# facebookresearch/seamless_communication

Measured on AMD Instinct MI355X. Metric: S2ST utterances/sec (and real-time factor), seamlessM4T_v2_large, 10 s audio, higher is better.
Workload: dtype f32 activations x f16 weights, f32 accumulate

## Files before the change

### seamless_communication_amd/csrc/k_attn.hip

```cpp
#include <cstdlib>

#include "kernels.h"

namespace sc {

static constexpr int HD = 64;

static constexpr int MQ = 128;
static constexpr int MKV = 32;
static constexpr int KS = 68;
typedef _Float16 a16_h8 __attribute__((ext_vector_type(8)));
typedef _Float16 a16_h4 __attribute__((ext_vector_type(4)));
static constexpr int KH_LD = 72;
static constexpr int VT_LD = 40;

__device__ __forceinline__ void a16_split8(const float* x, a16_h8& hi, a16_h8& lo) {
#pragma unroll
    for (int e = 0; e < 8; ++e) {
        const _Float16 h = (_Float16)x[e];
        hi[e] = h;
        lo[e] = (_Float16)(x[e] - (float)h);
    }
}

template <int MODE>
__global__ __launch_bounds__(256) void attn_mfma16_kernel(AttnArgs p) {
    constexpr bool SHAW = MODE == 1;
    constexpr bool RELPOS = MODE == 2;
    typedef float f16v __attribute__((ext_vector_type(16)));
    typedef float f4v __attribute__((ext_vector_type(4)));
    extern __shared__ __attribute__((aligned(16))) float smem[];
    _Float16* sKh = reinterpret_cast<_Float16*>(smem);
    _Float16* sKl = sKh + MKV * KH_LD;
    _Float16* sVh = sKl + MKV * KH_LD;
    _Float16* sVl = sVh + HD * VT_LD;
    float* sQR = smem + 4 * 32 * KS;
    float* sT = smem + 4 * 32 * KS;
    float* sR = smem;

    const int tid = threadIdx.x, lane = tid & 63, wave = tid >> 6;
    const int ql = lane & 31, hh = lane >> 5;
    int qb = blockIdx.x, h = blockIdx.y, n = blockIdx.z;
    {
        const int gx = gridDim.x, bh_all = gridDim.y * gridDim.z;
        if ((bh_all & 7) == 0) {
            const int L = blockIdx.x + gx * (blockIdx.y + gridDim.y * blockIdx.z);
            const int bh = (L / (8 * gx)) * 8 + (L & 7);
            qb = (L >> 3) % gx;
            h = bh % gridDim.y;
            n = bh / gridDim.y;
        }
    }
    const int q0 = qb * MQ + wave * 32;
    const int qi = q0 + ql;
    const int kv_len = p.kv_lens ? min(p.kv_lens[n], p.Skv) : p.Skv;
    const int shift = p.Skv - p.Sq;
    const int qabs = qi + shift;
    const int npos = p.rel_left + 1 + p.rel_right;
    const int sq_n = p.row_off ? kv_len : p.Sq;
    const int64_t qbase = p.row_off ? (int64_t)p.row_off[n] : (int64_t)n * p.Sq;
    const int64_t kvbase = p.row_off ? (int64_t)p.row_off[n] : (int64_t)n * p.Skv;
    if (p.row_off && qb * MQ >= kv_len) return;
    const bool qok = qi < sq_n;
    const float* qrow = p.q + (qbase + (qok ? qi : 0)) * p.ldq + h * HD;

    if (SHAW) {
        float qreg[32];
#pragma unroll
        for (int g = 0; g < 8; ++g) {
            f4v v = {0.f, 0.f, 0.f, 0.f};
            if (qok) v = *reinterpret_cast<const f4v*>(qrow + 8 * g + 4 * hh);
            qreg[4 * g + 0] = v[0];
            qreg[4 * g + 1] = v[1];
            qreg[4 * g + 2] = v[2];
            qreg[4 * g + 3] = v[3];
        }
        for (int idx = tid; idx < npos * (HD / 4); idx += 256) {
            const int r = idx >> 4, c4 = idx & 15;
            *reinterpret_cast<f4v*>(&sR[r * KS + c4 * 4]) = *reinterpret_cast<const f4v*>(p.rel_k + r * HD + c4 * 4);
        }
        __syncthreads();
#pragma unroll 1
        for (int f = 0; f < 3; ++f) {
            if (f * 32 >= npos) break;
            f16v qr;
#pragma unroll
            for (int r = 0; r < 16; ++r) qr[r] = 0.f;
#pragma unroll
            for (int g = 0; g < 8; ++g) {
                const f4v r4 = *reinterpret_cast<const f4v*>(&sR[(f * 32 + ql) * KS + 8 * g + 4 * hh]);
                qr = __builtin_amdgcn_mfma_f32_32x32x2f32(r4[0], qreg[4 * g + 0], qr, 0, 0, 0);
                qr = __builtin_amdgcn_mfma_f32_32x32x2f32(r4[1], qreg[4 * g + 1], qr, 0, 0, 0);
                qr = __builtin_amdgcn_mfma_f32_32x32x2f32(r4[2], qreg[4 * g + 2], qr, 0, 0, 0);
                qr = __builtin_amdgcn_mfma_f32_32x32x2f32(r4[3], qreg[4 * g + 3], qr, 0, 0, 0);
            }
#pragma unroll
            for (int r = 0; r < 16; ++r) {
                const int e = f * 32 + (r & 3) + 8 * (r >> 2) + 4 * hh;
                if (e < npos) sQR[(wave * 32 + ql) * npos + e] = qr[r];
            }
        }
    }

    a16_h8 qh[4], qlo[4], qvh[RELPOS ? 4 : 1], qvl[RELPOS ? 4 : 1];
#pragma unroll
    for (int c = 0; c < 4; ++c) {
        float x[8];
#pragma unroll
        for (int e = 0; e < 8; ++e) x[e] = 0.f;
        if (qok) {
            const f4v v0 = *reinterpret_cast<const f4v*>(qrow + 16 * c + 8 * hh);
            const f4v v1 = *reinterpret_cast<const f4v*>(qrow + 16 * c + 8 * hh + 4);
#pragma unroll
            for (int e = 0; e < 4; ++e) {
                x[e] = v0[e];
                x[4 + e] = v1[e];
            }
        }
        if (RELPOS) {
            float xu[8], xv[8];
#pragma unroll
            for (int e = 0; e < 8; ++e) {
                xu[e] = x[e] + p.q_bias_u[h * HD + 16 * c + 8 * hh + e];
                xv[e] = x[e] + p.q_bias_v[h * HD + 16 * c + 8 * hh + e];
            }
            a16_split8(xu, qh[c], qlo[c]);
            a16_split8(xv, qvh[c], qvl[c]);
        } else {
            a16_split8(x, qh[c], qlo[c]);
        }
    }

    f16v o0, o1;
#pragma unroll
    for (int r = 0; r < 16; ++r) {
        o0[r] = 0.f;
        o1[r] = 0.f;
    }
    float m_i = -1e30f, l_i = 0.f;

    int k_end = kv_len;
    if (p.causal) k_end = min(k_end, qb * MQ + MQ - 1 + shift + 1);

    const int sr0 = tid >> 4, sc4 = tid & 15;
    f4v kf[2], vf[2];
    auto fetch = [&](int k0) {
#pragma unroll
        for (int u = 0; u < 2; ++u) {
            const int r = sr0 + 16 * u;
            kf[u] = f4v{0.f, 0.f, 0.f, 0.f};
            vf[u] = kf[u];
            if (k0 + r < kv_len) {
                const int64_t row = kvbase + k0 + r;
                kf[u] = *reinterpret_cast<const f4v*>(p.k + row * p.ldk + h * HD + sc4 * 4);
                vf[u] = *reinterpret_cast<const f4v*>(p.v + row * p.ldv + h * HD + sc4 * 4);
            }
        }
    };
    if (k_end > 0) fetch(0);

    for (int k0 = 0; k0 < k_end; k0 += MKV) {
        __syncthreads();
#pragma unroll
        for (int u = 0; u < 2; ++u) {
            const int r = sr0 + 16 * u;
            a16_h4 khi, klo, vhi, vlo;
#pragma unroll
            for (int e = 0; e < 4; ++e) {
                const _Float16 a = (_Float16)kf[u][e];
                khi[e] = a;
                klo[e] = (_Float16)(kf[u][e] - (float)a);
                const _Float16 b = (_Float16)vf[u][e];
                vhi[e] = b;
                vlo[e] = (_Float16)(vf[u][e] - (float)b);
            }
            *reinterpret_cast<a16_h4*>(&sKh[r * KH_LD + 4 * sc4]) = khi;
            *reinterpret_cast<a16_h4*>(&sKl[r * KH_LD + 4 * sc4]) = klo;
            const int w = r & 15;
            const int pos = (r & 16) + 8 * ((w >> 2) & 1) + (w & 3) + 4 * (w >> 3);
#pragma unroll
            for (int e = 0; e < 4; ++e) {
                sVh[(4 * sc4 + e) * VT_LD + pos] = vhi[e];
                sVl[(4 * sc4 + e) * VT_LD + pos] = vlo[e];
            }
        }
        if (k0 + MKV < k_end) fetch(k0 + MKV);
        __syncthreads();

        float qr[16];
        if (SHAW) {
            const float* qrow_t = sQR + (wave * 32 + ql) * npos;
            const int rel_max = k0 + (MKV - 1) - (q0 + shift);
            const int rel_min = k0 - (q0 + 31 + shift);
            if (rel_max <= -p.rel_left) {
                const float v = qrow_t[0];
#pragma unroll
                for (int r = 0; r < 16; ++r) qr[r] = v;
            } else if (rel_min >= p.rel_right) {
                const float v = qrow_t[npos - 1];
#pragma unroll
                for (int r = 0; r < 16; ++r) qr[r] = v;
            } else {
#pragma unroll
                for (int r = 0; r < 16; ++r) {
                    const int kj = k0 + (r & 3) + 8 * (r >> 2) + 4 * hh;
                    const int rel = max(-p.rel_left, min(p.rel_right, kj - qabs)) + p.rel_left;
                    qr[r] = qrow_t[rel];
                }
            }
        }
        if (RELPOS) {
            const int t0w = (p.Skv - 1) - (q0 + shift) + k0 - 31;
            const int t_max = 2 * p.Skv - 2;
            float* tw = sT + wave * (64 * 32);
#pragma unroll
            for (int blk = 0; blk < 2; ++blk) {
                const int trow = min(max(t0w + blk * 32 + ql, 0), t_max);
                const float* rrow = p.rp_table + (int64_t)trow * p.rp_ld + h * HD + 8 * hh;
                f4v ra[4][2];
#pragma unroll
                for (int c = 0; c < 4; ++c) {
                    ra[c][0] = *reinterpret_cast<const f4v*>(rrow + 16 * c);
                    ra[c][1] = *reinterpret_cast<const f4v*>(rrow + 16 * c + 4);
                }
                f16v tt;
#pragma unroll
                for (int r = 0; r < 16; ++r) tt[r] = 0.f;
#pragma unroll
                for (int c = 0; c < 4; ++c) {
                    float x[8];
#pragma unroll
                    for (int e = 0; e < 4; ++e) {
                        x[e] = ra[c][0][e];
                        x[4 + e] = ra[c][1][e];
                    }
                    a16_h8 rh, rl;
                    a16_split8(x, rh, rl);
                    tt = __builtin_amdgcn_mfma_f32_32x32x16_f16(rh, qvh[c], tt, 0, 0, 0);
                    tt = __builtin_amdgcn_mfma_f32_32x32x16_f16(rh, qvl[c], tt, 0, 0, 0);
                    tt = __builtin_amdgcn_mfma_f32_32x32x16_f16(rl, qvh[c], tt, 0, 0, 0);
                }
#pragma unroll
                for (int r = 0; r < 16; ++r) tw[(blk * 32 + (r & 3) + 8 * (r >> 2) + 4 * hh) * 32 + ql] = tt[r];
            }
#pragma unroll
            for (int r = 0; r < 16; ++r) {
                const int jl = (r & 3) + 8 * (r >> 2) + 4 * hh;
                qr[r] = tw[(jl - ql + 31) * 32 + ql];
            }
        }
        f16v st;
#pragma unroll
        for (int r = 0; r < 16; ++r) st[r] = 0.f;
#pragma unroll
        for (int c = 0; c < 4; ++c) {
            const a16_h8 kh = *reinterpret_cast<const a16_h8*>(&sKh[ql * KH_LD + 16 * c + 8 * hh]);
            const a16_h8 kl = *reinterpret_cast<const a16_h8*>(&sKl[ql * KH_LD + 16 * c + 8 * hh]);
            st = __builtin_amdgcn_mfma_f32_32x32x16_f16(kh, qh[c], st, 0, 0, 0);
            st = __builtin_amdgcn_mfma_f32_32x32x16_f16(kh, qlo[c], st, 0, 0, 0);
            st = __builtin_amdgcn_mfma_f32_32x32x16_f16(kl, qh[c], st, 0, 0, 0);
        }
        float mx = -INFINITY;
#pragma unroll
        for (int r = 0; r < 16; ++r) {
            const int kj = k0 + (r & 3) + 8 * (r >> 2) + 4 * hh;
            float sc = st[r];
            if (SHAW || RELPOS) sc += qr[r];
            const bool ok = (kj < kv_len) && (!p.causal || kj <= qabs);
            sc = sc * 0.125f + (ok ? 0.f : -INFINITY);
            st[r] = sc;
            mx = fmaxf(mx, sc);
        }
        mx = fmaxf(mx, __shfl_xor(mx, 32));
        const float m_new = fmaxf(m_i, mx);
        constexpr float LOG2E = 1.44269504088896340736f;
        const float alpha = __builtin_amdgcn_exp2f((m_i - m_new) * LOG2E);
        float rs = 0.f;
#pragma unroll
        for (int r = 0; r < 16; ++r) {
            const float pv = __builtin_amdgcn_exp2f((st[r] - m_new) * LOG2E);
            st[r] = pv;
            rs += pv;
        }
        rs += __shfl_xor(rs, 32);
        l_i = l_i * alpha + rs;
        m_i = m_new;
        if (__builtin_amdgcn_ballot_w64(alpha != 1.f) != 0) {
#pragma unroll
            for (int r = 0; r < 16; ++r) {
                o0[r] *= alpha;
                o1[r] *= alpha;
            }
        }
#pragma unroll
        for (int c = 0; c < 2; ++c) {
            float x[8];
#pragma unroll
            for (int e = 0; e < 8; ++e) x[e] = st[8 * c + e];
            a16_h8 ph, pl;
            a16_split8(x, ph, pl);
            const a16_h8 v0h = *reinterpret_cast<const a16_h8*>(&sVh[ql * VT_LD + 16 * c + 8 * hh]);
            const a16_h8 v0l = *reinterpret_cast<const a16_h8*>(&sVl[ql * VT_LD + 16 * c + 8 * hh]);
            const a16_h8 v1h = *reinterpret_cast<const a16_h8*>(&sVh[(32 + ql) * VT_LD + 16 * c + 8 * hh]);
            const a16_h8 v1l = *reinterpret_cast<const a16_h8*>(&sVl[(32 + ql) * VT_LD + 16 * c + 8 * hh]);
            o0 = __builtin_amdgcn_mfma_f32_32x32x16_f16(v0h, ph, o0, 0, 0, 0);
            o1 = __builtin_amdgcn_mfma_f32_32x32x16_f16(v1h, ph, o1, 0, 0, 0);
            o0 = __builtin_amdgcn_mfma_f32_32x32x16_f16(v0h, pl, o0, 0, 0, 0);
            o1 = __builtin_amdgcn_mfma_f32_32x32x16_f16(v1h, pl, o1, 0, 0, 0);
            o0 = __builtin_amdgcn_mfma_f32_32x32x16_f16(v0l, ph, o0, 0, 0, 0);
            o1 = __builtin_amdgcn_mfma_f32_32x32x16_f16(v1l, ph, o1, 0, 0, 0);
        }
    }

    __syncthreads();
    float* ot = smem + wave * (32 * KS);
    const float inv = l_i > 0.f ? 1.0f / l_i : 0.f;
#pragma unroll
    for (int r = 0; r < 16; ++r) {
        const int d = (r & 3) + 8 * (r >> 2) + 4 * hh;
        ot[ql * KS + d] = o0[r] * inv;
        ot[ql * KS + 32 + d] = o1[r] * inv;
    }
#pragma unroll
    for (int it = 0; it < 8; ++it) {
        const int row = it * 4 + (lane >> 4);
        const int c0 = (lane & 15) * 4;
        const int qq = q0 + row;
        const f4v of = *reinterpret_cast<const f4v*>(&ot[row * KS + c0]);
        if (qq >= sq_n) continue;
        if (p.out_hi) {
            const a16_h4 hi = __builtin_convertvector(of, a16_h4);
            const f4v back = __builtin_convertvector(hi, f4v);
            const int64_t off = (qbase + qq) * p.ldoh + h * HD + c0;
            *reinterpret_cast<a16_h4*>(p.out_hi + off) = hi;
            *reinterpret_cast<a16_h4*>(p.out_lo + off) = __builtin_convertvector(of - back, a16_h4);
        } else {
            *reinterpret_cast<f4v*>(p.out + (qbase + qq) * p.ldo + h * HD + c0) = of;
        }
    }
}

static bool g_attn_attr_set = false;

void launch_attention(const AttnArgs& a, hipStream_t s) {
    if (a.head_dim == 80) {
        launch_attention80(a, s);
        return;
    }
    if (a.head_dim == 128) {
        launch_attention128(a, s);
        return;
    }
    SC_CHECK(a.head_dim == HD, "attention: head_dim=%d (64, 80 and 128 exist)", a.head_dim);
    SC_CHECK(a.nb > 0 && a.heads > 0 && a.Sq > 0 && a.Skv > 0, "attention: empty problem");
    SC_CHECK(a.out || (a.out_hi && a.out_lo && a.ldoh % 4 == 0), "attention: no output");
    SC_CHECK(a.ldq % 4 == 0 && a.ldk % 4 == 0 && a.ldv % 4 == 0 && a.ldo % 4 == 0 && (reinterpret_cast<uintptr_t>(a.out) & 15) == 0,
             "attention: row strides must be multiples of 4 and the output 16-byte aligned");
    const int npos = a.rel_left + 1 + a.rel_right;
    SC_CHECK(npos <= 96, "attention: %d relative positions > 96", npos);
    SC_CHECK(!a.row_off || (a.kv_lens && a.Sq == a.Skv && !a.causal), "attention: packed rows need kv_lens and Sq == Skv");
    if (a.rp_table)
        SC_CHECK(!a.rel_k && !a.causal && a.Sq == a.Skv && a.q_bias_u && a.q_bias_v && a.rp_ld % 4 == 0,
                 "attention: relative positions need self-attention (Sq == Skv), both query biases and a 16-byte aligned table");
    if (!g_attn_attr_set) {
        SC_HIP(hipFuncSetAttribute(reinterpret_cast<const void*>(&attn_mfma16_kernel<0>), hipFuncAttributeMaxDynamicSharedMemorySize, 120 * 1024));
        SC_HIP(hipFuncSetAttribute(reinterpret_cast<const void*>(&attn_mfma16_kernel<1>), hipFuncAttributeMaxDynamicSharedMemorySize, 120 * 1024));
        SC_HIP(hipFuncSetAttribute(reinterpret_cast<const void*>(&attn_mfma16_kernel<2>), hipFuncAttributeMaxDynamicSharedMemorySize, 120 * 1024));
        g_attn_attr_set = true;
    }
    const double pairs = a.pairs > 0 ? a.pairs : (double)a.nb * a.Sq * a.Skv;
    prof::Scope scope(a.rel_k ? "attention_shaw" : "attention", 4.0 * a.heads * pairs * HD,
                      4.0 * a.nb * a.heads * HD * (2.0 * a.Sq + 2.0 * a.Skv), s);
    size_t lds = (size_t)(4 * 32 * KS) * sizeof(float);
    if (a.rel_k) lds += (size_t)(MQ * npos) * sizeof(float);
    if (a.rp_table) lds += (size_t)(4 * 64 * 32) * sizeof(float);
    dim3 grid(cdiv(a.Sq, MQ), a.heads, a.nb);
    if (a.rp_table) hipLaunchKernelGGL((attn_mfma16_kernel<2>), grid, dim3(256), lds, s, a);
    else if (a.rel_k) hipLaunchKernelGGL((attn_mfma16_kernel<1>), grid, dim3(256), lds, s, a);
    else hipLaunchKernelGGL((attn_mfma16_kernel<0>), grid, dim3(256), lds, s, a);
    SC_LAUNCH_CHECK();
}

static constexpr int MAX_CACHE = 4096;

__global__ __launch_bounds__(256) void decode_attn_kernel(
    const float* __restrict__ q, int64_t ldq, const float* __restrict__ k_new,
    const float* __restrict__ v_new, int64_t ldkv, float* __restrict__ kcache,
    float* __restrict__ vcache, int64_t cache_ld, int64_t cache_bs, int cap, float* __restrict__ out,
    int64_t ldo, int heads, const int* __restrict__ d_pos, const int* __restrict__ kv_lens, int use_lens,
    int in_splits, int64_t in_split_stride, const float* __restrict__ bias_q,
    const float* __restrict__ bias_k, const float* __restrict__ bias_v) {
    __shared__ float s_q[HD];
    __shared__ float s_sc[MAX_CACHE];
    __shared__ float s_red[8];
    __shared__ float s_part[4][HD];

    const int tid = threadIdx.x, lane = tid & 63, wave = tid >> 6;
    const int h = blockIdx.x, b = blockIdx.y;
    const int pos = d_pos ? *d_pos : 0;
    const int kv_len = use_lens ? min(kv_lens[b], cap) : pos + 1;
    float* kc = kcache + (int64_t)b * cache_bs + h * HD;
    float* vc = vcache + (int64_t)b * cache_bs + h * HD;
    if (tid < 3 * HD) {
        const int which = tid >> 6, d = tid & 63;
        if (which == 0 || k_new) {
            const float* src = which == 0 ? q : (which == 1 ? k_new : v_new);
            const int64_t ld = which == 0 ? ldq : ldkv;
            const float* bias = which == 0 ? bias_q : (which == 1 ? bias_k : bias_v);
            float v = 0.f;
            for (int sp = 0; sp < in_splits; ++sp) v += src[(int64_t)sp * in_split_stride + (int64_t)b * ld + h * HD + d];
            if (bias) v += bias[h * HD + d];
            if (which == 0) s_q[d] = v;
            else if (which == 1) kc[(int64_t)pos * cache_ld + d] = v;
            else vc[(int64_t)pos * cache_ld + d] = v;
        }
    }
    __syncthreads();
    const int sub = lane & 15, grp = lane >> 4;
    const float4 q4 = *reinterpret_cast<const float4*>(&s_q[sub * 4]);
    float lmax = -INFINITY;
    for (int j0 = 0; j0 < kv_len; j0 += 16) {
        const int j = j0 + wave * 4 + grp;
        float d = 0.f;
        if (j < kv_len) {
            const float4 kv = *reinterpret_cast<const float4*>(kc + (int64_t)j * cache_ld + sub * 4);
            d = fmaf(q4.x, kv.x, d);
            d = fmaf(q4.y, kv.y, d);
            d = fmaf(q4.z, kv.z, d);
            d = fmaf(q4.w, kv.w, d);
        }
#pragma unroll
        for (int off = 8; off > 0; off >>= 1) d += __shfl_xor(d, off);
        if (j < kv_len) {
            d *= 0.125f;
            if (sub == 0) s_sc[j] = d;
            lmax = fmaxf(lmax, d);
        }
    }
#pragma unroll
    for (int off = 32; off > 0; off >>= 1) lmax = fmaxf(lmax, __shfl_xor(lmax, off));
    if (lane == 0) s_red[wave] = lmax;
    __syncthreads();
    const float mx = fmaxf(fmaxf(s_red[0], s_red[1]), fmaxf(s_red[2], s_red[3]));
    float lsum = 0.f;
    for (int j = tid; j < kv_len; j += 256) {
        const float e = expf(s_sc[j] - mx);
        s_sc[j] = e;
        lsum += e;
    }
#pragma unroll
    for (int off = 32; off > 0; off >>= 1) lsum += __shfl_xor(lsum, off);
    if (lane == 0) s_red[4 + wave] = lsum;
    __syncthreads();
    const float denom = (s_red[4] + s_red[5]) + (s_red[6] + s_red[7]);
    float acc = 0.f;
    for (int j = wave; j < kv_len; j += 4) acc = fmaf(s_sc[j], vc[(int64_t)j * cache_ld + lane], acc);
    s_part[wave][lane] = acc;
    __syncthreads();
    if (tid < HD) {
        const float v = (s_part[0][tid] + s_part[1][tid]) + (s_part[2][tid] + s_part[3][tid]);
        out[(int64_t)b * ldo + h * HD + tid] = v / denom;
    }
}

void launch_decode_attention(const float* q, int64_t ldq, const float* k_new, const float* v_new,
                             int64_t ldkv, float* kcache, float* vcache, int64_t cache_ld, int64_t cache_bs,
                             int cap, float* out, int64_t ldo, int nb, int heads, const int* d_pos,
                             const int* kv_lens, int use_lens, hipStream_t s, int in_splits,
                             int64_t in_split_stride, const float* bias_q, const float* bias_k,
                             const float* bias_v) {
    SC_CHECK(cap <= MAX_CACHE, "decode attention: cache capacity %d > %d", cap, MAX_CACHE);
    SC_CHECK(nb > 0 && heads > 0, "decode attention: empty problem");
    hipLaunchKernelGGL(decode_attn_kernel, dim3(heads, nb), dim3(256), 0, s, q, ldq, k_new, v_new, ldkv,
                       kcache, vcache, cache_ld, cache_bs, cap, out, ldo, heads, d_pos, kv_lens, use_lens,
                       in_splits < 1 ? 1 : in_splits, in_split_stride, bias_q, bias_k, bias_v);
    SC_LAUNCH_CHECK();
}

}
```

Baseline: 337.6.

## Split attention KV loop into unmasked interior and masked edge tiles

Turns the KV tile body into a lambda templated on an EDGE flag. Interior tiles, which lie entirely within kv_len and the causal bound, run without per-element masking and without bounds-checked prefetch, while only the trailing tiles pay for masking. It also packs the f32 to f16 hi/lo split into 2-wide vector conversions and makes the wave index uniform with readfirstlane. The cost is larger code and more complex loop-bound logic, where a boundary error would produce wrong masking.

```diff
diff --git a/seamless_communication_amd/csrc/k_attn.hip b/seamless_communication_amd/csrc/k_attn.hip
--- a/seamless_communication_amd/csrc/k_attn.hip
+++ b/seamless_communication_amd/csrc/k_attn.hip
@@ -1,4 +1,5 @@
 #include <cstdlib>
+#include <type_traits>
 
 #include "kernels.h"
 
@@ -14,12 +15,23 @@
 static constexpr int KH_LD = 72;
 static constexpr int VT_LD = 40;
 
+typedef float a16_f2 __attribute__((ext_vector_type(2)));
+typedef _Float16 a16_h2 __attribute__((ext_vector_type(2)));
+
+__device__ __forceinline__ void a16_split2(a16_f2 x, a16_h2& hi, a16_h2& lo) {
+    hi = __builtin_convertvector(x, a16_h2);
+    lo = __builtin_convertvector(x - __builtin_convertvector(hi, a16_f2), a16_h2);
+}
+
 __device__ __forceinline__ void a16_split8(const float* x, a16_h8& hi, a16_h8& lo) {
 #pragma unroll
-    for (int e = 0; e < 8; ++e) {
-        const _Float16 h = (_Float16)x[e];
-        hi[e] = h;
-        lo[e] = (_Float16)(x[e] - (float)h);
+    for (int e = 0; e < 8; e += 2) {
+        a16_h2 h, l;
+        a16_split2(a16_f2{x[e], x[e + 1]}, h, l);
+        hi[e] = h[0];
+        hi[e + 1] = h[1];
+        lo[e] = l[0];
+        lo[e + 1] = l[1];
     }
 }
 
@@ -38,7 +50,8 @@
     float* sT = smem + 4 * 32 * KS;
     float* sR = smem;
 
-    const int tid = threadIdx.x, lane = tid & 63, wave = tid >> 6;
+    const int tid = threadIdx.x, lane = tid & 63;
+    const int wave = __builtin_amdgcn_readfirstlane(tid >> 6);
     const int ql = lane & 31, hh = lane >> 5;
     int qb = blockIdx.x, h = blockIdx.y, n = blockIdx.z;
     {
@@ -144,35 +157,48 @@
 
     const int sr0 = tid >> 4, sc4 = tid & 15;
     f4v kf[2], vf[2];
-    auto fetch = [&](int k0) {
+    auto fetch = [&](auto edge, int k0) __attribute__((always_inline)) {
+        constexpr bool EDGE = decltype(edge)::value;
 #pragma unroll
         for (int u = 0; u < 2; ++u) {
             const int r = sr0 + 16 * u;
-            kf[u] = f4v{0.f, 0.f, 0.f, 0.f};
-            vf[u] = kf[u];
-            if (k0 + r < kv_len) {
+            if (EDGE) {
+                kf[u] = f4v{0.f, 0.f, 0.f, 0.f};
+                vf[u] = kf[u];
+            }
+            if (!EDGE || k0 + r < kv_len) {
                 const int64_t row = kvbase + k0 + r;
                 kf[u] = *reinterpret_cast<const f4v*>(p.k + row * p.ldk + h * HD + sc4 * 4);
                 vf[u] = *reinterpret_cast<const f4v*>(p.v + row * p.ldv + h * HD + sc4 * 4);
             }
         }
     };
-    if (k_end > 0) fetch(0);
-
-    for (int k0 = 0; k0 < k_end; k0 += MKV) {
+    if (k_end > 0) fetch(std::true_type{}, 0);
+
+    int k_int = kv_len;
+    if (p.causal) k_int = min(k_int, qb * MQ + shift + 1);
+    k_int = min(max(k_int, 0) & ~(MKV - 1), k_end);
+
+    auto tile = [&](auto edge, int k0) __attribute__((always_inline)) {
+        constexpr bool EDGE = decltype(edge)::value;
         __syncthreads();
 #pragma unroll
         for (int u = 0; u < 2; ++u) {
             const int r = sr0 + 16 * u;
             a16_h4 khi, klo, vhi, vlo;
 #pragma unroll
-            for (int e = 0; e < 4; ++e) {
-                const _Float16 a = (_Float16)kf[u][e];
-                khi[e] = a;
-                klo[e] = (_Float16)(kf[u][e] - (float)a);
-                const _Float16 b = (_Float16)vf[u][e];
-                vhi[e] = b;
-                vlo[e] = (_Float16)(vf[u][e] - (float)b);
+            for (int e = 0; e < 4; e += 2) {
+                a16_h2 a, b;
+                a16_split2(a16_f2{kf[u][e], kf[u][e + 1]}, a, b);
+                khi[e] = a[0];
+                khi[e + 1] = a[1];
+                klo[e] = b[0];
+                klo[e + 1] = b[1];
+                a16_split2(a16_f2{vf[u][e], vf[u][e + 1]}, a, b);
+                vhi[e] = a[0];
+                vhi[e + 1] = a[1];
+                vlo[e] = b[0];
+                vlo[e + 1] = b[1];
             }
             *reinterpret_cast<a16_h4*>(&sKh[r * KH_LD + 4 * sc4]) = khi;
             *reinterpret_cast<a16_h4*>(&sKl[r * KH_LD + 4 * sc4]) = klo;
@@ -184,7 +210,7 @@
                 sVl[(4 * sc4 + e) * VT_LD + pos] = vlo[e];
             }
         }
-        if (k0 + MKV < k_end) fetch(k0 + MKV);
+        if (!EDGE || k0 + MKV < k_end) fetch(edge, k0 + MKV);
         __syncthreads();
 
         float qr[16];
@@ -263,11 +289,15 @@
         float mx = -INFINITY;
 #pragma unroll
         for (int r = 0; r < 16; ++r) {
-            const int kj = k0 + (r & 3) + 8 * (r >> 2) + 4 * hh;
             float sc = st[r];
             if (SHAW || RELPOS) sc += qr[r];
-            const bool ok = (kj < kv_len) && (!p.causal || kj <= qabs);
-            sc = sc * 0.125f + (ok ? 0.f : -INFINITY);
+            if (EDGE) {
+                const int kj = k0 + (r & 3) + 8 * (r >> 2) + 4 * hh;
+                const bool ok = (kj < kv_len) && (!p.causal || kj <= qabs);
+                sc = sc * 0.125f + (ok ? 0.f : -INFINITY);
+            } else {
+                sc = sc * 0.125f;
+            }
             st[r] = sc;
             mx = fmaxf(mx, sc);
         }
@@ -310,7 +340,10 @@
             o0 = __builtin_amdgcn_mfma_f32_32x32x16_f16(v0l, ph, o0, 0, 0, 0);
             o1 = __builtin_amdgcn_mfma_f32_32x32x16_f16(v1l, ph, o1, 0, 0, 0);
         }
-    }
+    };
+    int k0 = 0;
+    for (; k0 + MKV < k_int; k0 += MKV) tile(std::false_type{}, k0);
+    for (; k0 < k_end; k0 += MKV) tile(std::true_type{}, k0);
 
     __syncthreads();
     float* ot = smem + wave * (32 * KS);
```

New measurement: 337.3. Within noise of the previous version (-0.1%).
